# shaofeifei11/SSDR-AL

Hardware: AMD Instinct MI355X
Metric: Mpoints/s subsample→KNN→RandLA-Net→FPS-GCN select, S3DIS 40960-pt tiles (higher is better)
Workload: dtype bf16x3: split-bf16 MFMA operands (hi*hi + lo*hi + hi*lo), fp32 accumulate, fp32 activations and non-matrix arithmetic

## Files before the change

### ssdr-al_amd/csrc/knn_grid.hip

```cpp
#include "ssdr_internal.hpp"
#include "block_prims.hpp"
#include "knn_regset.hpp"
#include <cfloat>
#include <cstring>

namespace ssdr {

namespace {

constexpr int GS_SAMPLES = 8;
constexpr int GS_BINS = 192;
constexpr int GS_BIN0 = (87 << 2);
constexpr int GS_RMAX = 3;
constexpr int SCAN_BLK = 4096;
constexpr float NEAR_TIE = 1.0000076293945312f;
constexpr int RETRY_FROM_R1 = 1 << 30;

__device__ __forceinline__ int cell_of(float v, float o, float inv_c, int n) {
    const float f = (v - o) * inv_c;
    int c = f > 0.f ? (int)fminf(f, 1.0e9f) : 0;
    return c < n ? c : n - 1;
}

constexpr int PREP_NT = 1024;
__global__ __launch_bounds__(PREP_NT) void grid_prepare_kernel(GridDesc* desc, int* cell, int target_pts) {
    __shared__ float s_mm[(PREP_NT / 64) * 6];
    __shared__ float s_smp[GS_SAMPLES][3];
    __shared__ int s_hist[GS_BINS];
    const int t = blockIdx.x, tid = threadIdx.x;
    GridDesc d = desc[t];
    const float* P = d.pts; const int n = d.n;
    float mn[3] = {FLT_MAX, FLT_MAX, FLT_MAX}, mx[3] = {-FLT_MAX, -FLT_MAX, -FLT_MAX};
    for (int i = tid; i < n; i += PREP_NT) {
        const float x = P[3 * (size_t)i], y = P[3 * (size_t)i + 1], z = P[3 * (size_t)i + 2];
        mn[0] = fminf(mn[0], x); mx[0] = fmaxf(mx[0], x); mn[1] = fminf(mn[1], y); mx[1] = fmaxf(mx[1], y); mn[2] = fminf(mn[2], z); mx[2] = fmaxf(mx[2], z);
    }
    block_minmax3<PREP_NT>(mn, mx, s_mm);
    for (int i = tid; i < GS_BINS; i += PREP_NT) s_hist[i] = 0;
    if (tid < GS_SAMPLES && n > 0) {
        const int i = (int)(((long long)tid * n) / GS_SAMPLES + n / (2 * GS_SAMPLES));
        s_smp[tid][0] = P[3 * (size_t)i]; s_smp[tid][1] = P[3 * (size_t)i + 1]; s_smp[tid][2] = P[3 * (size_t)i + 2];
    }
    __syncthreads();
    const int stride = n > 8192 ? n / 8192 : 1;
    for (int i = tid * stride; i < n; i += PREP_NT * stride) {
        const float x = P[3 * (size_t)i], y = P[3 * (size_t)i + 1], z = P[3 * (size_t)i + 2];
#pragma unroll
        for (int j = 0; j < GS_SAMPLES; ++j) {
            const float dx = x - s_smp[j][0], dy = y - s_smp[j][1], dz = z - s_smp[j][2];
            const float d2 = dx * dx + dy * dy + dz * dz;
            int b = (int)(__float_as_uint(d2) >> 21) - GS_BIN0;
            b = b < 0 ? 0 : (b >= GS_BINS ? GS_BINS - 1 : b);
            atomicAdd(&s_hist[b], 1);
        }
    }
    __syncthreads();
    if (tid == 0) {
        const float ex = mx[0] - mn[0], ey = mx[1] - mn[1], ez = mx[2] - mn[2];
        const float emax = fmaxf(ex, fmaxf(ey, ez));
        float c = emax > 0.f ? emax : 1.f;
        if (n > 4 * target_pts) {
            const long long want = ((long long)GS_SAMPLES * target_pts + stride - 1) / stride;
            long long cum = 0; int b = 0;
            for (; b < GS_BINS; ++b) { cum += s_hist[b]; if (cum >= want) break; }
            if (b < GS_BINS) {
                const float r2 = __uint_as_float((unsigned)(b + 1 + GS_BIN0) << 21);
                const float r = sqrtf(r2) * 1.1f;
                if (r > 0.f && r < c) c = r;
            }
        }
        for (int it = 0; it < 64; ++it) {
            const double cells = ((double)floorf(ex / c) + 1.0) * ((double)floorf(ey / c) + 1.0) * ((double)floorf(ez / c) + 1.0);
            if (cells <= (double)d.cell_cap) break;
            c *= 1.26f;
        }
        d.c = c; d.inv_c = 1.0f / c;
        d.nx = (int)floorf(ex / c) + 1; d.ny = (int)floorf(ey / c) + 1; d.nz = (int)floorf(ez / c) + 1;
        if ((long long)d.nx * d.ny * d.nz > d.cell_cap) { d.nx = d.ny = d.nz = 1; d.c = emax * 2.f + 1.f; d.inv_c = 1.0f / d.c; }
        d.ncell = d.nx * d.ny * d.nz;
        for (int k = 0; k < 3; ++k) { d.lo[k] = mn[k]; d.hi[k] = mx[k]; }
        if (n == 0) { d.nx = d.ny = d.nz = 1; d.ncell = 1; d.lo[0] = d.lo[1] = d.lo[2] = 0.f; d.c = 1.f; d.inv_c = 1.f; }
        {
            float mag = 0.f;
            for (int k = 0; k < 3; ++k) mag = fmaxf(mag, fmaxf(fabsf(d.lo[k]), fabsf(d.hi[k])));
            d.slack = 8.f * FLT_EPSILON * (2.f * mag + (float)(max(d.nx, max(d.ny, d.nz)) + 1) * d.c);
            d.pad_ = 0;
        }
        desc[t] = d;
        s_mm[0] = __int_as_float(d.ncell);
    }
    __syncthreads();
    const int ncell = __float_as_int(s_mm[0]);
    for (int i = tid; i <= ncell; i += PREP_NT) cell[d.cell_off + i] = 0;
}

__global__ __launch_bounds__(256) void grid_count_kernel(const GridDesc* __restrict__ desc, int* cell, int* __restrict__ rank) {
    const GridDesc d = desc[blockIdx.y];
    const int i = blockIdx.x * 256 + threadIdx.x;
    if (i >= d.n) return;
    const float x = d.pts[3 * (size_t)i], y = d.pts[3 * (size_t)i + 1], z = d.pts[3 * (size_t)i + 2];
    const int cid = (cell_of(z, d.lo[2], d.inv_c, d.nz) * d.ny + cell_of(y, d.lo[1], d.inv_c, d.ny)) * d.nx + cell_of(x, d.lo[0], d.inv_c, d.nx);
    rank[d.pt_off + i] = atomicAdd(&cell[d.cell_off + cid], 1);
}

__global__ __launch_bounds__(256) void grid_scan_sums_kernel(const GridDesc* __restrict__ desc, const int* __restrict__ cell, int* __restrict__ bsum, int max_blk) {
    __shared__ int s_part[4][2];
    const GridDesc d = desc[blockIdx.y];
    const int blk = blockIdx.x;
    if (blk * SCAN_BLK >= d.ncell) return;
    const int lo = blk * SCAN_BLK, hi = min(lo + SCAN_BLK, d.ncell);
    int s = 0, dummy = 0;
    for (int i = lo + threadIdx.x; i < hi; i += 256) s += cell[d.cell_off + i];
    block_sum2(s, dummy, &s_part[0][0]);
    if (threadIdx.x == 0) bsum[(size_t)blockIdx.y * max_blk + blk] = s;
}

__global__ __launch_bounds__(256) void grid_scan_apply_kernel(const GridDesc* __restrict__ desc, int* cell, const int* __restrict__ bsum, int max_blk) {
    __shared__ int s_wave[4];
    const GridDesc d = desc[blockIdx.y];
    const int blk = blockIdx.x, tid = threadIdx.x, lane = tid & 63, wid = tid >> 6;
    if (blk * SCAN_BLK >= d.ncell) return;
    int base = 0;
    for (int b = 0; b < blk; ++b) base += bsum[(size_t)blockIdx.y * max_blk + b];
    const int lo = blk * SCAN_BLK + tid * (SCAN_BLK / 256);
    int v[SCAN_BLK / 256]; int s = 0;
#pragma unroll
    for (int u = 0; u < SCAN_BLK / 256; ++u) { const int i = lo + u; v[u] = i < d.ncell ? cell[d.cell_off + i] : 0; s += v[u]; }
    int incl = s;
#pragma unroll
    for (int o = 1; o < 64; o <<= 1) { const int y = __shfl_up(incl, o); if (lane >= o) incl += y; }
    if (lane == 63) s_wave[wid] = incl;
    __syncthreads();
    int run = base + incl - s;
    for (int w2 = 0; w2 < wid; ++w2) run += s_wave[w2];
#pragma unroll
    for (int u = 0; u < SCAN_BLK / 256; ++u) { const int i = lo + u; if (i < d.ncell) cell[d.cell_off + i] = run; run += v[u]; }
    if (blk == (d.ncell - 1) / SCAN_BLK && tid == 0) cell[d.cell_off + d.ncell] = d.n;
}

__global__ __launch_bounds__(256) void grid_scatter_kernel(const GridDesc* __restrict__ desc, const int* __restrict__ cell, const int* __restrict__ rank,
                                                           float4* __restrict__ sorted) {
    const GridDesc d = desc[blockIdx.y];
    const int i = blockIdx.x * 256 + threadIdx.x;
    if (i >= d.n) return;
    const float x = d.pts[3 * (size_t)i], y = d.pts[3 * (size_t)i + 1], z = d.pts[3 * (size_t)i + 2];
    const int cid = (cell_of(z, d.lo[2], d.inv_c, d.nz) * d.ny + cell_of(y, d.lo[1], d.inv_c, d.ny)) * d.nx + cell_of(x, d.lo[0], d.inv_c, d.nx);
    sorted[d.pt_off + cell[d.cell_off + cid] + rank[d.pt_off + i]] = make_float4(x, y, z, __int_as_float(i));
}

struct GridSearchArgs {
    const GridDesc* desc; const int* cell; const float4* sorted; const GridJob* jobs; int job0;
    int* retry; int* retry_count;
    int* work; int* work_count; int work_cap; int* need; int* status;
    float4* ball_q; int* ball_tree; int* ball_count; float ball_scale;
};

template <int K>
__device__ __forceinline__ bool grid_settled(const GridDesc& d, float qx, float qy, float qz, int x0, int x1, int y0, int y1, int z0, int z1, const RegSet<K + 1>& rs) {
    float g = FLT_MAX;
    if (x0 > 0) g = fminf(g, qx - (d.lo[0] + (float)x0 * d.c));
    if (x1 < d.nx - 1) g = fminf(g, (d.lo[0] + (float)(x1 + 1) * d.c) - qx);
    if (y0 > 0) g = fminf(g, qy - (d.lo[1] + (float)y0 * d.c));
    if (y1 < d.ny - 1) g = fminf(g, (d.lo[1] + (float)(y1 + 1) * d.c) - qy);
    if (z0 > 0) g = fminf(g, qz - (d.lo[2] + (float)z0 * d.c));
    if (z1 < d.nz - 1) g = fminf(g, (d.lo[2] + (float)(z1 + 1) * d.c) - qz);
    if (g == FLT_MAX) return true;
    if (!(g > 0.f)) return false;
    const float gs = g * 0.99998f - d.slack;
    return gs > 0.f && rs.worst() <= gs * gs;
}

__device__ __forceinline__ float slab_gap(float q, float lo, float c, int i, int ci, float mg) {
    const float gap = i == ci ? 0.f : (i > ci ? (lo + (float)i * c) - q : q - (lo + (float)(i + 1) * c));
    return fmaxf(gap - mg, 0.f);
}

template <int K, typename OutT>
__device__ __forceinline__ void grid_finish(const GridSearchArgs& a, const GridJob& job, int jid, int q, bool settled, const RegSet<K + 1>& rs) {
    bool hard = !settled || rs.d[K] == FLT_MAX;
    const bool unsettled = hard;
#pragma unroll
    for (int j = 0; j < K; ++j) hard |= rs.d[j] == rs.d[j + 1];
    hard |= rs.d[K] <= rs.d[K - 1] * NEAR_TIE;
    if (hard) {
        if (unsettled) atomicAdd(a.status + 1, 1);
        const int w = atomicAdd(a.work_count, 1);
        if (w < a.work_cap) { a.work[2 * (size_t)w] = jid; a.work[2 * (size_t)w + 1] = q; a.need[job.sup] = 1; }
        else atomicOr(a.status, 8);
        const int bi = atomicAdd(a.ball_count, 1);
        if (bi < GRID_BALL_CAP) {
            const float* qp = job.qpts + 3 * (size_t)q;
            a.ball_q[bi] = make_float4(qp[0], qp[1], qp[2], unsettled ? FLT_MAX : rs.d[K] * a.ball_scale);
            a.ball_tree[bi] = job.sup;
        }
        return;
    }
    OutT* o = reinterpret_cast<OutT*>(job.out) + (size_t)q * K;
#pragma unroll
    for (int j = 0; j < K; ++j) o[j] = (OutT)rs.id[j];
}

struct SrcGlobal { const float4* S; __device__ __forceinline__ float4 operator()(int, int, int i) const { return S[i]; } };
struct SrcLds {
    const float4* S; const float4* lds; const int* delta; int z0, y0, nys; bool staged;
    __device__ __forceinline__ float4 operator()(int z, int y, int i) const { return staged ? lds[i + delta[(z - z0) * nys + (y - y0)]] : S[i]; }
};
template <int K, int R, class Src>
__device__ __forceinline__ int grid_mark_select(const GridDesc& d, const int* __restrict__ cell, const Src S, float qx, float qy, float qz,
                                                RegSet<K + 1>& rs, int n1, float& b0, float& b1, int& i0, float& tau) {
    constexpr int W = 2 * R + 1;
    const int cx = cell_of(qx, d.lo[0], d.inv_c, d.nx), cy = cell_of(qy, d.lo[1], d.inv_c, d.ny), cz = cell_of(qz, d.lo[2], d.inv_c, d.nz);
    const int x0 = max(cx - R, 0), x1 = min(cx + R, d.nx - 1);
    float g = FLT_MAX;
    if (x0 > 0) g = fminf(g, qx - (d.lo[0] + (float)x0 * d.c));
    if (x1 < d.nx - 1) g = fminf(g, (d.lo[0] + (float)(x1 + 1) * d.c) - qx);
    if (cy - R > 0) g = fminf(g, qy - (d.lo[1] + (float)(cy - R) * d.c));
    if (cy + R < d.ny - 1) g = fminf(g, (d.lo[1] + (float)(cy + R + 1) * d.c) - qy);
    if (cz - R > 0) g = fminf(g, qz - (d.lo[2] + (float)(cz - R) * d.c));
    if (cz + R < d.nz - 1) g = fminf(g, (d.lo[2] + (float)(cz + R + 1) * d.c) - qz);
    if (!(g > 0.f)) return 2;
    tau = FLT_MAX;
    if (g < FLT_MAX) { const float gs = g * 0.99998f - d.slack; if (!(gs > 0.f)) return 2; tau = gs * gs; }
    unsigned long long m[W * W]; int rs0[W * W];
    int cnt = 0; bool long_row = false;
#pragma unroll
    for (int r = 0; r < W * W; ++r) {
        const int z = cz + r / W - R, y = cy + r % W - R;
        m[r] = 0ull; rs0[r] = 0;
        if (z < 0 || z >= d.nz || y < 0 || y >= d.ny) continue;
        const int row = (z * d.ny + y) * d.nx;
        const int s = cell[row + x0], e = cell[row + x1 + 1];
        rs0[r] = s;
        if (e - s > 64) { long_row = true; continue; }
        for (int i = s; i < e; i += 4) {
            float4 p[4];
#pragma unroll
            for (int u = 0; u < 4; ++u) p[u] = S(z, y, min(i + u, e - 1));
#pragma unroll
            for (int u = 0; u < 4; ++u) {
                const float dx = qx - p[u].x, dy = qy - p[u].y, dz = qz - p[u].z;
                float dist = dx * dx; dist = dist + dy * dy; dist = dist + dz * dz;
                if (i + u < e && dist < tau) { m[r] |= 1ull << (i + u - s); ++cnt; }
            }
        }
    }
    if (long_row) return 2;
    if (cnt < K + 1) {
        if (n1 > 0) {
#pragma unroll
            for (int r = 0; r < W * W; ++r) {
                unsigned long long mm = m[r];
                while (mm) {
                    const int bpos = __ffsll((unsigned long long)mm) - 1;
                    mm &= mm - 1ull;
                    const float4 p = S(cz + r / W - R, cy + r % W - R, rs0[r] + bpos);
                    const float dx = qx - p.x, dy = qy - p.y, dz = qz - p.z;
                    float dist = dx * dx; dist = dist + dy * dy; dist = dist + dz * dz;
                    if (__float_as_int(p.w) < n1 && dist < b1) { if (dist < b0) { b1 = b0; b0 = dist; i0 = __float_as_int(p.w); } else b1 = dist; }
                }
            }
        }
        return 1;
    }
    rs.init();
#pragma unroll
    for (int r = 0; r < W * W; ++r) {
        unsigned long long mm = m[r];
        while (mm) {
            const int bpos = __ffsll((unsigned long long)mm) - 1;
            mm &= mm - 1ull;
            const float4 p = S(cz + r / W - R, cy + r % W - R, rs0[r] + bpos);
            const float dx = qx - p.x, dy = qy - p.y, dz = qz - p.z;
            float dist = dx * dx; dist = dist + dy * dy; dist = dist + dz * dz;
            const int id = __float_as_int(p.w);
            if (id < n1 && dist < b1) { if (dist < b0) { b1 = b0; b0 = dist; i0 = id; } else b1 = dist; }
            if (dist < rs.worst()) rs.add(dist, id);
        }
    }
    return 0;
}

template <int K, typename OutT, class Src>
__device__ __forceinline__ void grid_search_query(const GridSearchArgs& a, const GridJob& job, int jid, const GridDesc& d, const Src src, int q, float qx, float qy, float qz) {
    RegSet<K + 1> rs;
    float b0 = FLT_MAX, b1 = FLT_MAX, tau = 0.f; int i0 = 0;
    const bool fuse1 = K == 16 && job.job1 >= 0;
    const int st = grid_mark_select<K, 1>(d, a.cell + d.cell_off, src, qx, qy, qz, rs, fuse1 ? job.n1 : 0, b0, b1, i0, tau);
    if (fuse1) {
        if (st != 2 && b0 < tau && b0 * NEAR_TIE < fminf(b1, tau)) {
            const GridJob j1 = a.jobs[job.job1];
            reinterpret_cast<OutT*>(j1.out)[q] = (OutT)i0;
        } else {
            const int w = atomicAdd(a.retry_count + 1, 1);
            int* r1 = a.retry + 2 * (size_t)a.work_cap;
            r1[2 * (size_t)w] = job.job1 | RETRY_FROM_R1; r1[2 * (size_t)w + 1] = q;
        }
    }
    if (st != 0) {
        const int w = atomicAdd(a.retry_count, 1);
        a.retry[2 * (size_t)w] = st == 2 ? (jid | RETRY_FROM_R1) : jid; a.retry[2 * (size_t)w + 1] = q;
        return;
    }
    grid_finish<K, OutT>(a, job, jid, q, true, rs);
}

template <int K, typename OutT>
__global__ __launch_bounds__(256) SSDR_WAVES_PER_EU(5) void grid_search_kernel(GridSearchArgs a) {
    int bx, by; xcd_tile_map(bx, by);
    const int jid = a.job0 + by;
    const GridJob job = a.jobs[jid];
    const int qi = bx * 256 + (int)threadIdx.x;
    if (qi >= job.nq) return;
    const GridDesc d = a.desc[job.sup];
    int q = qi; float qx, qy, qz;
    if (job.ord >= 0) {
        const float4 r = a.sorted[a.desc[job.ord].pt_off + qi];
        q = __float_as_int(r.w); qx = r.x; qy = r.y; qz = r.z;
    } else {
        qx = job.qpts[3 * (size_t)q]; qy = job.qpts[3 * (size_t)q + 1]; qz = job.qpts[3 * (size_t)q + 2];
    }
    grid_search_query<K, OutT>(a, job, jid, d, SrcGlobal{a.sorted + d.pt_off}, q, qx, qy, qz);
}

constexpr int GL_CAP = 2048, GL_ROWS = 96;
template <int K, typename OutT>
__global__ __launch_bounds__(256) void grid_search_lds_kernel(GridSearchArgs a) {
    __shared__ float4 s_rec[GL_CAP];
    __shared__ int s_delta[GL_ROWS], s_start[GL_ROWS], s_len[GL_ROWS], s_mm[4], s_tot;
    int bx, by; xcd_tile_map(bx, by);
    const int jid = a.job0 + by;
    const GridJob job = a.jobs[jid];
    const int tid = threadIdx.x, lane = tid & 63, wid = tid >> 6;
    const int qi = bx * 256 + tid;
    const bool live = qi < job.nq;
    const GridDesc d = a.desc[job.sup];
    int q = qi; float qx = 0.f, qy = 0.f, qz = 0.f;
    if (live) {
        if (job.ord >= 0) { const float4 r = a.sorted[a.desc[job.ord].pt_off + qi]; q = __float_as_int(r.w); qx = r.x; qy = r.y; qz = r.z; }
        else { qx = job.qpts[3 * (size_t)q]; qy = job.qpts[3 * (size_t)q + 1]; qz = job.qpts[3 * (size_t)q + 2]; }
    }
    if (tid == 0) { s_mm[0] = 0x7fffffff; s_mm[1] = -1; s_mm[2] = 0x7fffffff; s_mm[3] = -1; }
    __syncthreads();
    if (live) {
        const int cy = cell_of(qy, d.lo[1], d.inv_c, d.ny), cz = cell_of(qz, d.lo[2], d.inv_c, d.nz);
        atomicMin(&s_mm[0], cz); atomicMax(&s_mm[1], cz); atomicMin(&s_mm[2], cy); atomicMax(&s_mm[3], cy);
    }
    __syncthreads();
    if (s_mm[1] < 0) return;
    const int z0 = max(s_mm[0] - 1, 0), z1 = min(s_mm[1] + 1, d.nz - 1), y0 = max(s_mm[2] - 1, 0), y1 = min(s_mm[3] + 1, d.ny - 1);
    const int nys = y1 - y0 + 1, nrows = (z1 - z0 + 1) * nys;
    const int* cell = a.cell + d.cell_off;
    const float4* S = a.sorted + d.pt_off;
    bool staged = nrows > 0 && nrows <= GL_ROWS;
    if (staged) {
        if (tid < nrows) { const int row = ((z0 + tid / nys) * d.ny + (y0 + tid % nys)) * d.nx; const int gs = cell[row]; s_start[tid] = gs; s_len[tid] = cell[row + d.nx] - gs; }
        __syncthreads();
        if (tid == 0) { int run = 0; for (int r = 0; r < nrows; ++r) { s_delta[r] = run - s_start[r]; run += s_len[r]; } s_tot = run; }
        __syncthreads();
        staged = s_tot <= GL_CAP;
        if (staged)
            for (int r = wid; r < nrows; r += 4)
                for (int i = lane; i < s_len[r]; i += 64) s_rec[s_delta[r] + s_start[r] + i] = S[s_start[r] + i];
        __syncthreads();
    }
    if (!live) return;
    grid_search_query<K, OutT>(a, job, jid, d, SrcLds{S, s_rec, s_delta, z0, y0, nys, staged}, q, qx, qy, qz);
}

constexpr int RL = 8, RCB = 64;
template <int K, typename OutT>
__global__ __launch_bounds__(64) void grid_retry_kernel(GridSearchArgs a) {
    constexpr int RPW = 64 / RL;
    __shared__ float c_d[RPW][RCB];
    __shared__ int c_i[RPW][RCB];
    __shared__ int c_n[RPW];
    __shared__ float s_gw[RPW];
    __shared__ int s_set[RPW];
    const int lane = threadIdx.x, sub = lane % RL, grp = lane / RL;
    const int n = min(*a.retry_count, a.work_cap);
    for (int e0 = blockIdx.x * RPW; e0 < n; e0 += gridDim.x * RPW) {
        const bool live = e0 + grp < n;
        const int e = min(e0 + grp, n - 1);
        const int tag = a.retry[2 * (size_t)e], q = a.retry[2 * (size_t)e + 1];
        const int jid = tag & ~RETRY_FROM_R1;
        const GridJob job = a.jobs[jid];
        const GridDesc d = a.desc[job.sup];
        const int* __restrict__ cell = a.cell + d.cell_off;
        const float4* __restrict__ S = a.sorted + d.pt_off;
        const float qx = job.qpts[3 * (size_t)q], qy = job.qpts[3 * (size_t)q + 1], qz = job.qpts[3 * (size_t)q + 2];
        const int cx = cell_of(qx, d.lo[0], d.inv_c, d.nx), cy = cell_of(qy, d.lo[1], d.inv_c, d.ny), cz = cell_of(qz, d.lo[2], d.inv_c, d.nz);
        RegSet<K + 1> G;
        G.init();
        float gw = FLT_MAX; bool settled = false;
        const float mg = d.c * 1.0e-3f + 1.0e-6f * fmaxf(fmaxf(fabsf(qx), fabsf(qy)), fabsf(qz));
        if (sub == 0) c_n[grp] = 0;
        auto drain = [&]() {
            wave_sync();
            if (sub == 0) {
                const int m = c_n[grp];
                for (int j = 0; j < m; ++j) { const float dist = c_d[grp][j]; if (dist < G.worst()) G.add(dist, c_i[grp][j]); }
                c_n[grp] = 0; s_gw[grp] = G.worst();
            }
            wave_sync();
            gw = s_gw[grp];
        };
        for (int R = 1; R <= GS_RMAX; ++R) {
            const int x0 = max(cx - R, 0), x1 = min(cx + R, d.nx - 1), y0 = max(cy - R, 0), y1 = min(cy + R, d.ny - 1), z0 = max(cz - R, 0), z1 = min(cz + R, d.nz - 1);
            const int W = 2 * R + 1;
            const float r = sqrtf(gw) * 1.00001f + mg;
            const float r2 = r * r;
            const int zs = max(z0, cell_of(qz - r, d.lo[2], d.inv_c, d.nz)), ze = min(z1, cell_of(qz + r, d.lo[2], d.inv_c, d.nz));
            const int ix0 = cx - (R - 1), ix1 = cx + (R - 1);
            for (int t0 = 0; t0 < W * W; t0 += RL) {
                const int t = t0 + sub;
                int cs[2] = {1, 1}, ce[2] = {0, 0}, row = 0;
                if (!settled && t < W * W) {
                    const int z = cz - R + t / W, y = cy - R + t % W;
                    const float gz = slab_gap(qz, d.lo[2], d.c, z, cz, mg);
                    const float remz = r2 - gz * gz;
                    if (z >= zs && z <= ze && remz > 0.f) {
                        const float hy = sqrtf(remz);
                        const int ys = max(y0, cell_of(qy - hy, d.lo[1], d.inv_c, d.ny)), ye = min(y1, cell_of(qy + hy, d.lo[1], d.inv_c, d.ny));
                        const float gy = slab_gap(qy, d.lo[1], d.c, y, cy, mg);
                        const float rem = remz - gy * gy;
                        if (y >= ys && y <= ye && rem > 0.f) {
                            const float h = sqrtf(rem);
                            const int xs = max(x0, cell_of(qx - h, d.lo[0], d.inv_c, d.nx)), xe = min(x1, cell_of(qx + h, d.lo[0], d.inv_c, d.nx));
                            row = (z * d.ny + y) * d.nx;
                            const bool inner = R > 1 && abs(z - cz) < R && abs(y - cy) < R;
                            cs[0] = xs; ce[0] = inner ? min(xe + 1, ix0) : xe + 1;
                            if (inner) { cs[1] = max(xs, ix1 + 1); ce[1] = xe + 1; }
                        }
                    }
                }
#pragma unroll
                for (int u = 0; u < 2; ++u) {
                    int i = 0, e1 = 0;
                    if (cs[u] < ce[u]) { i = cell[row + cs[u]]; e1 = cell[row + ce[u]]; }
                    while (__ballot(i < e1)) {
                        wave_sync();
                        if (__ballot(c_n[grp] > RCB - 4 * RL)) drain();
                        if (i < e1) {
                            float4 p[4];
#pragma unroll
                            for (int v = 0; v < 4; ++v) p[v] = S[min(i + v, e1 - 1)];
#pragma unroll
                            for (int v = 0; v < 4; ++v) {
                                const float dx = qx - p[v].x, dy = qy - p[v].y, dz = qz - p[v].z;
                                float dist = dx * dx; dist = dist + dy * dy; dist = dist + dz * dz;
                                if (i + v < e1 && dist < gw) { const int pos = atomicAdd(&c_n[grp], 1); c_d[grp][pos] = dist; c_i[grp][pos] = __float_as_int(p[v].w); }
                            }
                            i += 4;
                        }
                    }
                }
            }
            drain();
            if (sub == 0 && !settled) s_set[grp] = grid_settled<K>(d, qx, qy, qz, x0, x1, y0, y1, z0, z1, G) ? 1 : 0;
            wave_sync();
            if (!settled) settled = s_set[grp] != 0;
            wave_sync();
            if (__ballot(!settled) == 0ull) break;
        }
        if (sub == 0 && live) grid_finish<K, OutT>(a, job, jid, q, settled, G);
    }
}

}

int grid_build(GridForest& g, const std::vector<GridDesc>& sets_in, int target_pts, hipStream_t s) {
    std::vector<GridDesc> sets = sets_in;
    long pt = 0, cl = 0; int maxn = 0; long maxcap = 0;
    for (auto& d : sets) {
        d.pt_off = (int)pt; d.cell_off = (int)cl; d.cell_cap = 8 * d.n + 64;
        pt += d.n; cl += (long)d.cell_cap + 1; maxn = std::max(maxn, d.n); maxcap = std::max(maxcap, (long)d.cell_cap);
        if (pt > 0x3fffffffL || cl > 0x7ffffff0L) { set_error("grid_build: too many points"); return SSDR_ERR_INVALID; }
    }
    g.nsets = (int)sets.size(); g.total_pts = (int)pt; g.max_n = maxn;
    g.max_blk = (int)((maxcap + SCAN_BLK - 1) / SCAN_BLK);
    if (g.nsets == 0) return SSDR_OK;
    SSDR_TRY(g.desc.reserve(sizeof(GridDesc) * sets.size()));
    SSDR_TRY(g.cell.reserve(4 * (size_t)cl + 16)); SSDR_TRY(g.rank.reserve(4 * (size_t)std::max(pt, 1L))); SSDR_TRY(g.sorted.reserve(16 * (size_t)std::max(pt, 1L)));
    SSDR_TRY(g.bsum.reserve(4 * (size_t)g.nsets * g.max_blk));
    SSDR_TRY(g.need.reserve(4 * (2 * (size_t)g.nsets + 16)));
    SSDR_TRY(g.balls.reserve((size_t)GRID_BALL_CAP * 20));
    {
        GridDesc* st = nullptr;
        const int slot = g.staging.acquire(sets.size(), &st);
        if (slot < 0) { set_error("grid_build: pinned staging buffer"); return SSDR_ERR_HIP; }
        memcpy(st, sets.data(), sizeof(GridDesc) * sets.size());
        SSDR_HIP(hipMemcpyAsync(g.desc.p, st, sizeof(GridDesc) * sets.size(), hipMemcpyHostToDevice, s));
        if (g.staging.release(slot, s)) { set_error("grid_build: staging event"); return SSDR_ERR_HIP; }
    }
    SSDR_HIP(hipMemsetAsync(g.need.p, 0, 4 * (2 * (size_t)g.nsets + 16), s));
    GridDesc* dd = g.desc.as<GridDesc>();
    const dim3 gp((unsigned)((maxn + 255) / 256), (unsigned)g.nsets), gb((unsigned)g.max_blk, (unsigned)g.nsets);
    ProfScope prof("knn_grid_build", s, 28.0 * (double)pt);
    hipLaunchKernelGGL(grid_prepare_kernel, dim3(g.nsets), dim3(PREP_NT), 0, s, dd, g.cell.as<int>(), target_pts);
    hipLaunchKernelGGL(grid_count_kernel, gp, dim3(256), 0, s, dd, g.cell.as<int>(), g.rank.as<int>());
    hipLaunchKernelGGL(grid_scan_sums_kernel, gb, dim3(256), 0, s, dd, g.cell.as<int>(), g.bsum.as<int>(), g.max_blk);
    hipLaunchKernelGGL(grid_scan_apply_kernel, gb, dim3(256), 0, s, dd, g.cell.as<int>(), g.bsum.as<int>(), g.max_blk);
    hipLaunchKernelGGL(grid_scatter_kernel, gp, dim3(256), 0, s, dd, g.cell.as<int>(), g.rank.as<int>(), g.sorted.as<float4>());
    SSDR_HIP(hipGetLastError());
    return SSDR_OK;
}

int grid_search(const GridForest& g, int job0, int njobs, int max_nq, int K, bool out_i64, hipStream_t s, double prof_bytes) {
    if (njobs <= 0) return SSDR_OK;
    if (K != 16 && K != 1) { set_error("grid search: K=%d has no instantiation (1, 16)", K); return SSDR_ERR_UNSUPPORTED; }
    const int wl = K == 16 ? 0 : 1;
    int* ctr = g.counters();
    GridSearchArgs a{g.desc.as<GridDesc>(), g.cell.as<int>(), g.sorted.as<float4>(), g.jobs.as<GridJob>(), job0,
                     g.work_list(2 + wl), ctr + 4 + wl, g.work_list(wl), ctr + wl, g.work_cap, g.need.as<int>(), ctr + 2,
                     g.ball_q(), g.ball_tree(), ctr + 6, g.ball_scale};
    const dim3 grid((unsigned)((max_nq + 255) / 256), (unsigned)njobs);
    const dim3 rgrid((unsigned)std::max(1, std::min(g.work_cap / 64 + 1, ctx().num_cu * 16)));
    const bool first = max_nq > 0;
    static const bool lds_form = [] { const char* e = getenv("SSDR_KNN_LDS"); return e && e[0] == '1'; }();
    if (first) {
        ProfScope prof(K == 16 ? "grid_search_kernel<16>" : "grid_search_kernel<1>", s, prof_bytes);
        if (K == 16) {
            if (out_i64) { if (lds_form) hipLaunchKernelGGL((grid_search_lds_kernel<16, int64_t>), grid, dim3(256), 0, s, a); else hipLaunchKernelGGL((grid_search_kernel<16, int64_t>), grid, dim3(256), 0, s, a); }
            else { if (lds_form) hipLaunchKernelGGL((grid_search_lds_kernel<16, int32_t>), grid, dim3(256), 0, s, a); else hipLaunchKernelGGL((grid_search_kernel<16, int32_t>), grid, dim3(256), 0, s, a); }
        } else {
            if (out_i64) hipLaunchKernelGGL((grid_search_kernel<1, int64_t>), grid, dim3(256), 0, s, a);
            else hipLaunchKernelGGL((grid_search_kernel<1, int32_t>), grid, dim3(256), 0, s, a);
        }
    }
    {
        ProfScope prof(K == 16 ? "grid_retry_kernel<16>" : "grid_retry_kernel<1>", s, first ? 0.0 : prof_bytes);
        if (K == 16) { if (out_i64) hipLaunchKernelGGL((grid_retry_kernel<16, int64_t>), rgrid, dim3(64), 0, s, a); else hipLaunchKernelGGL((grid_retry_kernel<16, int32_t>), rgrid, dim3(64), 0, s, a); }
        else { if (out_i64) hipLaunchKernelGGL((grid_retry_kernel<1, int64_t>), rgrid, dim3(64), 0, s, a); else hipLaunchKernelGGL((grid_retry_kernel<1, int32_t>), rgrid, dim3(64), 0, s, a); }
    }
    SSDR_HIP(hipGetLastError());
    return SSDR_OK;
}

int grid_set_jobs(GridForest& g, const std::vector<GridJob>& jobs, hipStream_t s) {
    if (jobs.empty()) return SSDR_OK;
    long tq = 0; for (auto& j : jobs) tq += j.nq;
    g.work_cap = (int)std::min(std::max(tq, 1024L), 0x3fffffffL);
    SSDR_TRY(g.work.reserve(4 * 8 * (size_t)g.work_cap));
    SSDR_TRY(g.jobs.reserve(sizeof(GridJob) * jobs.size()));
    {
        GridJob* st = nullptr;
        const int slot = g.jstaging.acquire(jobs.size(), &st);
        if (slot < 0) { set_error("grid_set_jobs: pinned staging buffer"); return SSDR_ERR_HIP; }
        memcpy(st, jobs.data(), sizeof(GridJob) * jobs.size());
        SSDR_HIP(hipMemcpyAsync(g.jobs.p, st, sizeof(GridJob) * jobs.size(), hipMemcpyHostToDevice, s));
        if (g.jstaging.release(slot, s)) { set_error("grid_set_jobs: staging event"); return SSDR_ERR_HIP; }
    }
    return SSDR_OK;
}

}
```

Baseline: 204.2.

## Spill per-row KNN candidate masks to LDS and prefetch points in gather loop

```diff
diff --git a/ssdr-al_amd/csrc/knn_grid.hip b/ssdr-al_amd/csrc/knn_grid.hip
--- a/ssdr-al_amd/csrc/knn_grid.hip
+++ b/ssdr-al_amd/csrc/knn_grid.hip
@@ -200,16 +200,17 @@
     for (int j = 0; j < K; ++j) o[j] = (OutT)rs.id[j];
 }
 
-struct SrcGlobal { const float4* S; __device__ __forceinline__ float4 operator()(int, int, int i) const { return S[i]; } };
+struct SrcGlobal { const float4* S; unsigned* mk; __device__ __forceinline__ float4 operator()(int, int, int i) const { return S[i]; } };
 struct SrcLds {
     const float4* S; const float4* lds; const int* delta; int z0, y0, nys; bool staged;
     __device__ __forceinline__ float4 operator()(int z, int y, int i) const { return staged ? lds[i + delta[(z - z0) * nys + (y - y0)]] : S[i]; }
 };
-template <int K, int R, class Src>
-__device__ __forceinline__ int grid_mark_select(const GridDesc& d, const int* __restrict__ cell, const Src S, float qx, float qy, float qz,
-                                                RegSet<K + 1>& rs, int n1, float& b0, float& b1, int& i0, float& tau) {
+template <int R, class Src, class Sink>
+__device__ __forceinline__ int grid_mark_rows(const GridDesc& d, const int* __restrict__ cell, const Src S, float qx, float qy, float qz,
+                                              int& cy, int& cz, float& tau, int& cnt, Sink sink) {
     constexpr int W = 2 * R + 1;
-    const int cx = cell_of(qx, d.lo[0], d.inv_c, d.nx), cy = cell_of(qy, d.lo[1], d.inv_c, d.ny), cz = cell_of(qz, d.lo[2], d.inv_c, d.nz);
+    const int cx = cell_of(qx, d.lo[0], d.inv_c, d.nx);
+    cy = cell_of(qy, d.lo[1], d.inv_c, d.ny); cz = cell_of(qz, d.lo[2], d.inv_c, d.nz);
     const int x0 = max(cx - R, 0), x1 = min(cx + R, d.nx - 1);
     float g = FLT_MAX;
     if (x0 > 0) g = fminf(g, qx - (d.lo[0] + (float)x0 * d.c));
@@ -221,17 +222,15 @@
     if (!(g > 0.f)) return 2;
     tau = FLT_MAX;
     if (g < FLT_MAX) { const float gs = g * 0.99998f - d.slack; if (!(gs > 0.f)) return 2; tau = gs * gs; }
-    unsigned long long m[W * W]; int rs0[W * W];
-    int cnt = 0; bool long_row = false;
+    cnt = 0; bool long_row = false;
 #pragma unroll
     for (int r = 0; r < W * W; ++r) {
         const int z = cz + r / W - R, y = cy + r % W - R;
-        m[r] = 0ull; rs0[r] = 0;
         if (z < 0 || z >= d.nz || y < 0 || y >= d.ny) continue;
         const int row = (z * d.ny + y) * d.nx;
         const int s = cell[row + x0], e = cell[row + x1 + 1];
-        rs0[r] = s;
         if (e - s > 64) { long_row = true; continue; }
+        unsigned long long m = 0ull;
         for (int i = s; i < e; i += 4) {
             float4 p[4];
 #pragma unroll
@@ -240,29 +239,76 @@
             for (int u = 0; u < 4; ++u) {
                 const float dx = qx - p[u].x, dy = qy - p[u].y, dz = qz - p[u].z;
                 float dist = dx * dx; dist = dist + dy * dy; dist = dist + dz * dz;
-                if (i + u < e && dist < tau) { m[r] |= 1ull << (i + u - s); ++cnt; }
+                if (i + u < e && dist < tau) { m |= 1ull << (i + u - s); ++cnt; }
             }
         }
-    }
-    if (long_row) return 2;
-    if (cnt < K + 1) {
-        if (n1 > 0) {
-#pragma unroll
-            for (int r = 0; r < W * W; ++r) {
-                unsigned long long mm = m[r];
-                while (mm) {
-                    const int bpos = __ffsll((unsigned long long)mm) - 1;
-                    mm &= mm - 1ull;
-                    const float4 p = S(cz + r / W - R, cy + r % W - R, rs0[r] + bpos);
-                    const float dx = qx - p.x, dy = qy - p.y, dz = qz - p.z;
-                    float dist = dx * dx; dist = dist + dy * dy; dist = dist + dz * dz;
-                    if (__float_as_int(p.w) < n1 && dist < b1) { if (dist < b0) { b1 = b0; b0 = dist; i0 = __float_as_int(p.w); } else b1 = dist; }
-                }
+        sink(r, m, s);
+    }
+    return long_row ? 2 : 0;
+}
+
+constexpr int GM_NT = 256;
+template <int R> constexpr int grid_mark_words() { return (2 * R + 1) * (2 * R + 1) * 3 * GM_NT; }
+template <int K, int R>
+__device__ __forceinline__ int grid_mark_select(const GridDesc& d, const int* __restrict__ cell, const SrcGlobal S, float qx, float qy, float qz,
+                                                RegSet<K + 1>& rs, int n1, float& b0, float& b1, int& i0, float& tau) {
+    constexpr int W = 2 * R + 1;
+    static_assert(W * W <= 32, "one bit per row of cells");
+    unsigned* const mk = S.mk;
+    unsigned ne = 0u;
+    int cy, cz, cnt;
+    const int st = grid_mark_rows<R>(d, cell, S, qx, qy, qz, cy, cz, tau, cnt, [&](int r, unsigned long long m, int s) {
+        if (m) { ne |= 1u << r; mk[(3 * r) * GM_NT] = (unsigned)m; mk[(3 * r + 1) * GM_NT] = (unsigned)(m >> 32); mk[(3 * r + 2) * GM_NT] = (unsigned)s; }
+    });
+    if (st) return st;
+    const bool full = cnt >= K + 1;
+    int left = full || n1 > 0 ? cnt : 0;
+    if (full) rs.init();
+    if (left > 0) {
+        int nr = __builtin_ctz(ne), r = 0, idx = 0;
+        ne &= ne - 1u;
+        unsigned long long mm = 0ull, nmm; int base = 0, nbase;
+        auto next = [&](bool want) {
+            const bool adv = want && mm == 0ull;
+            if (adv) { mm = nmm; base = nbase; r = nr; }
+            if (adv && ne) {
+                nr = __builtin_ctz(ne); ne &= ne - 1u;
+                nmm = (unsigned long long)mk[(3 * nr) * GM_NT] | ((unsigned long long)mk[(3 * nr + 1) * GM_NT] << 32);
+                nbase = (int)mk[(3 * nr + 2) * GM_NT];
             }
-        }
-        return 1;
-    }
-    rs.init();
+            if (want) { idx = base + __ffsll((unsigned long long)mm) - 1; mm &= mm - 1ull; }
+        };
+        nmm = (unsigned long long)mk[(3 * nr) * GM_NT] | ((unsigned long long)mk[(3 * nr + 1) * GM_NT] << 32);
+        nbase = (int)mk[(3 * nr + 2) * GM_NT];
+        next(true);
+        float4 pf = S(cz + r / W - R, cy + r % W - R, idx);
+        do {
+            const float4 p = pf;
+            const float dx = qx - p.x, dy = qy - p.y, dz = qz - p.z;
+            float dist = dx * dx; dist = dist + dy * dy; dist = dist + dz * dz;
+            const int id = __float_as_int(p.w);
+            next(left > 1);
+            pf = S(cz + r / W - R, cy + r % W - R, idx);
+            if (id < n1 && dist < b1) { if (dist < b0) { b1 = b0; b0 = dist; i0 = id; } else b1 = dist; }
+            if (full && dist < rs.worst()) rs.add(dist, id);
+        } while (--left > 0);
+    }
+    return full ? 0 : 1;
+}
+
+template <int K, int R>
+__device__ __forceinline__ int grid_mark_select(const GridDesc& d, const int* __restrict__ cell, const SrcLds S, float qx, float qy, float qz,
+                                                RegSet<K + 1>& rs, int n1, float& b0, float& b1, int& i0, float& tau) {
+    constexpr int W = 2 * R + 1;
+    unsigned long long m[W * W]; int rs0[W * W];
+#pragma unroll
+    for (int r = 0; r < W * W; ++r) { m[r] = 0ull; rs0[r] = 0; }
+    int cy, cz, cnt;
+    const int st = grid_mark_rows<R>(d, cell, S, qx, qy, qz, cy, cz, tau, cnt, [&](int r, unsigned long long mr, int s) { m[r] = mr; rs0[r] = s; });
+    if (st) return st;
+    const bool full = cnt >= K + 1;
+    if (!full && n1 <= 0) return 1;
+    if (full) rs.init();
 #pragma unroll
     for (int r = 0; r < W * W; ++r) {
         unsigned long long mm = m[r];
@@ -274,10 +320,10 @@
             float dist = dx * dx; dist = dist + dy * dy; dist = dist + dz * dz;
             const int id = __float_as_int(p.w);
             if (id < n1 && dist < b1) { if (dist < b0) { b1 = b0; b0 = dist; i0 = id; } else b1 = dist; }
-            if (dist < rs.worst()) rs.add(dist, id);
-        }
-    }
-    return 0;
+            if (full && dist < rs.worst()) rs.add(dist, id);
+        }
+    }
+    return full ? 0 : 1;
 }
 
 template <int K, typename OutT, class Src>
@@ -305,11 +351,12 @@
 }
 
 template <int K, typename OutT>
-__global__ __launch_bounds__(256) SSDR_WAVES_PER_EU(5) void grid_search_kernel(GridSearchArgs a) {
+__global__ __launch_bounds__(GM_NT) SSDR_WAVES_PER_EU(5) void grid_search_kernel(GridSearchArgs a) {
+    __shared__ unsigned s_mark[grid_mark_words<1>()];
     int bx, by; xcd_tile_map(bx, by);
     const int jid = a.job0 + by;
     const GridJob job = a.jobs[jid];
-    const int qi = bx * 256 + (int)threadIdx.x;
+    const int qi = bx * GM_NT + (int)threadIdx.x;
     if (qi >= job.nq) return;
     const GridDesc d = a.desc[job.sup];
     int q = qi; float qx, qy, qz;
@@ -319,7 +366,7 @@
     } else {
         qx = job.qpts[3 * (size_t)q]; qy = job.qpts[3 * (size_t)q + 1]; qz = job.qpts[3 * (size_t)q + 2];
     }
-    grid_search_query<K, OutT>(a, job, jid, d, SrcGlobal{a.sorted + d.pt_off}, q, qx, qy, qz);
+    grid_search_query<K, OutT>(a, job, jid, d, SrcGlobal{a.sorted + d.pt_off, s_mark + threadIdx.x}, q, qx, qy, qz);
 }
 
 constexpr int GL_CAP = 2048, GL_ROWS = 96;
@@ -520,11 +567,11 @@
     if (first) {
         ProfScope prof(K == 16 ? "grid_search_kernel<16>" : "grid_search_kernel<1>", s, prof_bytes);
         if (K == 16) {
-            if (out_i64) { if (lds_form) hipLaunchKernelGGL((grid_search_lds_kernel<16, int64_t>), grid, dim3(256), 0, s, a); else hipLaunchKernelGGL((grid_search_kernel<16, int64_t>), grid, dim3(256), 0, s, a); }
-            else { if (lds_form) hipLaunchKernelGGL((grid_search_lds_kernel<16, int32_t>), grid, dim3(256), 0, s, a); else hipLaunchKernelGGL((grid_search_kernel<16, int32_t>), grid, dim3(256), 0, s, a); }
+            if (out_i64) { if (lds_form) hipLaunchKernelGGL((grid_search_lds_kernel<16, int64_t>), grid, dim3(GM_NT), 0, s, a); else hipLaunchKernelGGL((grid_search_kernel<16, int64_t>), grid, dim3(GM_NT), 0, s, a); }
+            else { if (lds_form) hipLaunchKernelGGL((grid_search_lds_kernel<16, int32_t>), grid, dim3(GM_NT), 0, s, a); else hipLaunchKernelGGL((grid_search_kernel<16, int32_t>), grid, dim3(GM_NT), 0, s, a); }
         } else {
-            if (out_i64) hipLaunchKernelGGL((grid_search_kernel<1, int64_t>), grid, dim3(256), 0, s, a);
-            else hipLaunchKernelGGL((grid_search_kernel<1, int32_t>), grid, dim3(256), 0, s, a);
+            if (out_i64) hipLaunchKernelGGL((grid_search_kernel<1, int64_t>), grid, dim3(GM_NT), 0, s, a);
+            else hipLaunchKernelGGL((grid_search_kernel<1, int32_t>), grid, dim3(GM_NT), 0, s, a);
         }
     }
     {
```

Result: faster. 207.1, median of 6 (+1.4%).
